# IIT-PAVIS/Acoustic-Image-Generation

Hardware: AMD Instinct MI355X
Metric: train-step images/sec (higher is better)
Workload: dtype f32

## Files before the change

### acoustic-image-generation_amd/acimg/_lib.py

```python
import ctypes as C
import os

_HERE = os.path.dirname(os.path.abspath(__file__))
LIB_PATH = os.environ.get("ACIMG_LIB") or os.path.join(_HERE, "lib", "libacimg.so")

ACT_NONE, ACT_RELU, ACT_SIGMOID = 0, 1, 2


class ConvDesc(C.Structure):

    _fields_ = [(n, C.c_int32) for n in (
        "N", "H", "W", "C", "ldx", "K", "ldy", "OH", "OW", "R", "S", "stride", "pad_t", "pad_l",
        "ldw", "act")]

    def __repr__(self):
        return "ConvDesc(" + ", ".join("%s=%d" % (n, getattr(self, n)) for n, _ in self._fields_) + ")"


class Config(C.Structure):

    _fields_ = [(n, C.c_int32) for n in (
        "splitk_cut", "splitk_target", "splitk_handoff", "wgrad_minpix", "wgrad_halo", "split3_tile_bm",
        "split3_tile_bn", "tail_split", "tail_s", "trunk_persistent", "trunk_bk", "trunk_stagger", "trunk_dma_pos",
        "trunk_ring", "trunk_ring_bm", "trunk_halo")]
# ... 26 lines not shown
    "acimg_last_error": (_I, [C.c_char_p, _SZ]),
    "acimg_conv2d_fwd": (_I, [_DP, _P, _P, _P, _P, _P, _P, _I, _P, _P, _SZ, _P, _P]),
    "acimg_conv2d_stats_rows": (_I, [_DP]),
    "acimg_conv2d_fwd_tiling": (_I, [_DP, C.POINTER(C.c_int)]),
    "acimg_config_default": (_I, [C.POINTER(Config)]),
    "acimg_configure": (_I, [C.POINTER(Config)]),
    "acimg_conv2d_fwd_workspace": (_SZ, [_DP]),
    "acimg_conv2d_split3_weight_bytes": (_SZ, [_DP]),
    "acimg_conv2d_split3_prepare": (_I, [_DP, _P, _P, _P]),
    "acimg_conv2d_bf16_prepare": (_I, [_DP, _P, _P, _P]),
    "acimg_conv2d_fwd_split3_stats_rows": (_I, [_DP]),
    "acimg_conv2d_fwd_split3_tiling": (_I, [_DP, C.POINTER(C.c_int)]),
    "acimg_conv2d_fwd_split3p_stats_rows": (_I, [_DP]),
    "acimg_conv2d_fwd_split3": (_I, [_DP, _P, _P, _P, _P, _P, _P, _I, _P, _P]),
    "acimg_conv2d_fwd_bf16": (_I, [_DP, _P, _P, _P, _P, _P, _P, _I, _P, _P]),
    "acimg_conv2d_split3_dgrad_weight_bytes": (_SZ, [_DP]),
    "acimg_conv2d_split3_prepare_dgrad": (_I, [_DP, _P, _P, _P]),
    "acimg_conv2d_dgrad_split3": (_I, [_DP, _P, _I, _P, _P, _I, _P, _I, _P, _I, _P]),
    "acimg_conv2d_dgrad_bf16": (_I, [_DP, _P, _I, _P, _P, _I, _P, _I, _P, _I, _P]),
    "acimg_conv2d_split3_prepare_multi": (_I, [_I, _P, _P, _P, _P, _P]),
    "acimg_conv2d_fwd_split3p_workspace": (_SZ, [_DP]),
    "acimg_conv2d_fwd_split3p": (_I, [_DP, _P, _SZ, _P, _P, _P, _P, _SZ, _P]),
    "acimg_conv2d_fwd_split1p": (_I, [_DP, _P, _SZ, _P, _P, _P, _P, _SZ, _P]),
    "acimg_conv2d_fwd_split3p_stats": (_I, [_DP, _P, _SZ, _P, _P, _P, _SZ, _P]),
    "acimg_gram_stats_workspace": (_SZ, [_L, _I]),
    "acimg_gram_stats": (_I, [_P, _SZ, _L, _I, _P, _I, _I, _P, _P, _P, _P, _F, _F, _P, _P, _P, _SZ, _P]),
    "acimg_conv2d_fwd_split3p_tail": (_I, [_DP, _P, _SZ, _P, _P, _P, _P, _SZ, _P, _SZ, _P, _SZ, _P]),
    "acimg_conv2d_fwd_split3p_tail_proj": (_I, [_DP, _P, _SZ, _P, _P, _P, _P, _P, _P, _P, _SZ, _P, _SZ, _P]),
    "acimg_split_plane_bytes": (_SZ, [_L, _I]),
    "acimg_bn_relu_split": (_I, [_P, _P, _P, _I, _P, _SZ, _L, _I, _P]),
    "acimg_bn_add_relu_split": (_I, [_P, _P, _P, _P, _P, _P, _P, _SZ, _P, _SZ, _P, _I, _I, _I, _I, _I, _I, _I, _P]),
    "acimg_bn_relu_maxpool_split": (_I, [_P, _P, _P, _P, _SZ, _I, _I, _I, _I, _I, _I, _I, _I, _P]),
    "acimg_conv2d_dgrad": (_I, [_DP, _P, _I, _P, _P, _I, _P, _I, _P, _I, _P, _SZ, _P, _P]),
    "acimg_conv2d_dgrad_workspace": (_SZ, [_DP]),
    "acimg_conv2d_wgrad": (_I, [_DP, _P, _P, _I, _P, _P, _P, _SZ, _P]),
    "acimg_conv2d_wgrad_workspace": (_SZ, [_DP]),
    "acimg_conv2d_wgrad_split3": (_I, [_DP, _P, _P, _I, _P, _P, _P, _SZ, _P]),
    "acimg_conv2d_wgrad_bf16": (_I, [_DP, _P, _P, _I, _P, _P, _P, _SZ, _P]),
    "acimg_conv2d_affine_input_ok": (_I, [_DP, _I]),
    "acimg_conv2d_wgrad_affine": (_I, [_DP, _I, _P, _P, _P, _I, _P, _I, _P, _P, _P, _SZ, _P]),
    "acimg_deconv_fwd": (_I, [_DP, _P, _P, _P, _P, _P, _SZ, _P, _P]),
    "acimg_deconv_dgrad": (_I, [_DP, _P, _I, _P, _P, _P, _I, _P, _SZ, _P, _P]),
    "acimg_deconv_wgrad": (_I, [_DP, _P, _P, _I, _P, _P, _P, _SZ, _P]),
    "acimg_deconv_workspace": (_SZ, [_DP]),
    "acimg_bn_finalize": (_I, [_P, _I, _I, _I, _D, _P, _P, _P, _P, _F, _F, _I, _P, _P, _P, _P, _P]),
    "acimg_bn_add_relu": (_I, [_P, _P, _P, _P, _P, _P, _P, _I, _I, _I, _I, _I, _I, _I, _P]),
# ... 134 lines not shown
```

### acoustic-image-generation_amd/acimg/ops.py

```python
import ctypes as C
import math

import torch

from . import _lib
from ._lib import ACT_NONE, ACT_RELU, ACT_SIGMOID, ConvDesc


def up4(v):
    return (int(v) + 3) & ~3


class Ptr(object):

    __slots__ = ("t", "off")

    def __init__(self, t, off=0):
        self.t = t
        self.off = int(off)

    def addr(self):
        return self.t.data_ptr() + 4 * self.off


# ... 404 lines not shown

def conv2d_fwd_split3(plan, d, x, wsplit, y, in_scale=None, in_shift=None, in_relu=0, stats=None, bias=None, bf16=False):
    fn = _L().acimg_conv2d_fwd_bf16 if bf16 else _L().acimg_conv2d_fwd_split3
    _check_stats_rows(stats, _L().acimg_conv2d_fwd_split3_stats_rows(C.byref(d)), "conv2d_fwd_split3")
    plan.add("conv2d_fwd_bf16" if bf16 else "conv2d_fwd_split3", fn, C.byref(d), x, wsplit, bias, y, in_scale, in_shift,
             int(in_relu), stats)


def conv2d_split3_dgrad_weight_bytes(d):
    return _L().acimg_conv2d_split3_dgrad_weight_bytes(C.byref(d))


def conv2d_split3_prepare_dgrad(plan, d, w, wsplit):
    plan.add("conv2d_split3_prepare_dgrad", _L().acimg_conv2d_split3_prepare_dgrad, C.byref(d), w, wsplit)


def conv2d_dgrad_split3(plan, d, gy, ldgy, wsplit_t, dx, residual=None, ldres=0, mask=None, ldmask=0, lddx=0,
                        bf16=False):
    fn = _L().acimg_conv2d_dgrad_bf16 if bf16 else _L().acimg_conv2d_dgrad_split3
    plan.add("conv2d_dgrad_bf16" if bf16 else "conv2d_dgrad_split3", fn, C.byref(d), gy, int(ldgy), wsplit_t, dx,
             int(lddx), residual, int(ldres), mask, int(ldmask))


def conv2d_fwd_split3p_workspace(d):
    return int(_L().acimg_conv2d_fwd_split3p_workspace(C.byref(d)))


def conv2d_fwd_split3p(plan, d, x_planes, x_lo_off, wsplit, y, stats=None, tail_ws=None, terms=3, side=False):
    nbytes = 0 if tail_ws is None else (tail_ws.numel() * tail_ws.element_size() if hasattr(tail_ws, "numel") else 0)
    fn = _L().acimg_conv2d_fwd_split3p if terms == 3 else _L().acimg_conv2d_fwd_split1p
    plan.add("conv2d_fwd_split3p" if terms == 3 else "conv2d_fwd_split1p", fn, C.byref(d), x_planes, int(x_lo_off),
             wsplit, y, stats, tail_ws, int(nbytes), side=side)


def conv2d_fwd_split3p_stats(plan, d, x_planes, x_lo_off, wsplit, stats, tail_ws=None, side=False):
    nbytes = 0 if tail_ws is None else (tail_ws.numel() * tail_ws.element_size() if hasattr(tail_ws, "numel") else 0)
    plan.add("conv2d_fwd_split3p_stats", _L().acimg_conv2d_fwd_split3p_stats, C.byref(d), x_planes, int(x_lo_off), wsplit,
             stats, tail_ws, int(nbytes), side=side)


def gram_stats_workspace(rows, Cn):
    return int(_L().acimg_gram_stats_workspace(int(rows), int(Cn)))


def gram_stats(plan, x_planes, x_lo_off, rows, Cn, w, ldw, K, gamma, beta, moving_mean, moving_var, scale, shift, ws,
               decay=0.997, eps=1e-5, side=False):
    plan.add("gram_stats", _L().acimg_gram_stats, x_planes, int(x_lo_off), int(rows), int(Cn), w, int(ldw), int(K), gamma,
             beta, moving_mean, moving_var, float(decay), float(eps), scale, shift, ws,
             int(ws.numel() * ws.element_size()), side=side)


def conv2d_fwd_split3p_tail(plan, d, x_planes, x_lo_off, wsplit, scale, shift, sc_planes, sc_lo_off, out_planes,
                            out_lo_off, tail_ws=None, side=False):
    nbytes = 0 if tail_ws is None else (tail_ws.numel() * tail_ws.element_size() if hasattr(tail_ws, "numel") else 0)
    plan.add("conv2d_fwd_split3p_tail", _L().acimg_conv2d_fwd_split3p_tail, C.byref(d), x_planes, int(x_lo_off), wsplit,
             scale, shift, sc_planes, int(sc_lo_off), out_planes, int(out_lo_off), tail_ws, int(nbytes), side=side)

# ... 324 lines not shown
```

### acoustic-image-generation_amd/acimg/unet_acresnet.py

```python
import os
from collections import OrderedDict

import numpy as np
import torch

from . import ops
from .ops import ACT_NONE, ACT_RELU, ACT_SIGMOID, Ptr
from .params import FusedHeads, Var, up4
from .session import get_default_session
from .vision import load_state_file

Z = 150


class Act(object):

    def __init__(self, t, N, H, W, C, ld=None, off=0):
        self.t, self.N, self.H, self.W, self.C = t, N, H, W, C
        self.ld = up4(C) if ld is None else ld
        self.off = off

    @property
    def ptr(self):
        return Ptr(self.t, self.off)

    @property
    def Cp(self):
        return up4(self.C)

    @property
    def pixels(self):
        return self.N * self.H * self.W


class UNetAc(object):

    def __init__(self, input_shape=None, num_frames=12, embedding=False, num_skip=1, precision="split", side_lane=True):
        assert precision in ("split", "f32")
        self.precision = precision
        self.split_min_rows = 16384
        self.side_lane = bool(side_lane)
        self._wsplit_bufs = {}
        self.scope = 'UNetAcRes'
        self.num_frames = num_frames
        self.height = input_shape[0]
        self.width = input_shape[1]
        self.channels = input_shape[2]
        self.embedding = bool(embedding)
        self.num_skip = int(num_skip)
        assert self.num_skip in (0, 1, 2)
        self.session = None

    def _conv_specs(self):
        ns = self.num_skip
        return OrderedDict([
            ("final", (3, 3, 64, 12)),
            ("layer7/conv_2", (3, 3, 64, 64)), ("layer7/conv_1", (3, 3, 128, 64)),
            ("layer6/conv_2", (3, 3, 128, 128)), ("layer6/conv_1", (3, 3, 128 if ns == 0 else 256, 128)),
            ("layer5/conv_2", (3, 3, 128, 128)), ("layer5/conv_1", (3, 3, 128, 128)),
            ("layer4/conv_2", (3, 3, 128, 128)), ("layer4/conv_1", (3, 3, 266 if ns == 2 else 133, 128)),
            ("conv2d", (3, 3, 12, 133)),
            ("layer2/conv_2", (3, 3, 133, 133)), ("layer2/conv_1", (3, 3, 128, 133)),
            ("layer1/pool_2", (3, 3, 128, 128)), ("layer1/conv_2", (3, 3, 128, 128)),
# ... 110 lines not shown
        else:
            self.mean = self.zbuf[:, :Z]
        self.output = self.yhat.t
        self.network = OrderedDict(input=acoustic_images, is_training=None, keep_prob=None,
                                   features=self.cat145[..., :145])
        self.train_vars = [n for n in sess.store.tf_names() if n.startswith(self.scope + "/")]

    def _P(self, name):
        st = self.session.store
        return ops.LazyPtr(lambda: st.p(self.scope + "/" + name))

    def _G(self, name):
        st = self.session.store
        return ops.LazyPtr(lambda: st.g(self.scope + "/" + name))

    def _desc(self, x, K, stride=1, y=None, act=ACT_NONE):
        return ops.conv_desc(x.N, x.H, x.W, x.Cp if x.off == 0 and x.ld == x.Cp else x.C, K, 3, 3, stride, "SAME",
                             ldx=x.ld, ldy=(y.ld if y is not None else up4(K)), ldw=up4(K), act=act)

    def _use_split(self, d):
        return (self.precision == "split" and d.stride == 1 and d.C % 32 == 0 and d.K % 32 == 0 and
                d.N * d.OH * d.OW >= self.split_min_rows)

    def _wsplit(self, name, nbytes, kind):
        key = (name, kind)
        if key not in self._wsplit_bufs:
            self._wsplit_bufs[key] = torch.zeros(int(nbytes), dtype=torch.uint8, device=self.session.device)
        return self._wsplit_bufs[key]

    def _prepare_job(self, plan, d, name, image, mode):
        if getattr(self, "_prep_jobs", None) is None:
            (ops.conv2d_split3_prepare_dgrad if mode else ops.conv2d_split3_prepare)(plan, d, self._P(name + "/kernel"),
                                                                                      image)
            return
        self._prep_jobs.add(d, self._P(name + "/kernel"), image, mode)

    def _conv(self, plan, name, x, y, stride=1, act=ACT_RELU):
        d = self._desc(x, y.C, stride, y, act)
        self._descs[name] = (d, x, y)
        if self._use_split(d):
            ws = self._wsplit(name, ops.conv2d_split3_weight_bytes(d), "fwd")
            self._prepare_job(plan, d, name, ws, 0)
            ops.conv2d_fwd_split3(plan, d, x.ptr, ws, y.ptr, bias=self._P(name + "/bias"))
        else:
            ops.conv2d_fwd(plan, d, x.ptr, self._P(name + "/kernel"), self._P(name + "/bias"), y.ptr)

    def _record_forward(self, plan):
        N = self.N
        self._descs = {}
        h, w = self.pool1.H, self.pool1.W
        self._prep_jobs = None
        if self.precision == "split":
            self._prep_jobs = ops.PrepareJobs()
            ops.conv2d_split3_prepare_multi(plan, self._prep_jobs)
        self._conv(plan, "layer1/conv_1", self.inp, self.c11)
        self._conv(plan, "layer1/conv_2", self.c11, self.conv1)
        self._conv(plan, "layer1/pool_2", self.conv1, self.pool1, stride=3)
        self._conv(plan, "layer2/conv_1", self.pool1, self.c21)
        self._conv(plan, "layer2/conv_2", self.c21, self.conv2_0)
        ops.minmax_fwd(plan, self.conv2_0.ptr, self.conv2_0.ld, self.cat145, 148, self.mm_a, N, h * w, 133)
        ops.minmax_fwd(plan, self.feat.ptr, 12, Ptr(self.cat145, 133), 148, self.mm_b, N, h * w, 12)
        kin = h * w * 148
        self.d_heads = ops.conv_desc(N, 1, 1, kin, self.hn if not self.embedding else Z, 1, 1, 1, "VALID",
                                     ldx=kin, ldy=self.hn, ldw=self.hn)
        ops.conv2d_fwd(plan, self.d_heads, self.cat145, self._P("heads/kernel"), self._P("heads/bias"),
                       self.heads_out)
        if self.embedding:
            ops.minmax_fwd(plan, self.heads_out, self.hn, self.zbuf, 152, self.mm_z, N, 1, Z)
        else:
            ops.latent_fwd(plan, self.heads_out, self.eps, self.zbuf, 152, self.sigma, self.kl, N, Z)
        self.d_dense = ops.conv_desc(N, 1, 1, 152, 2304, 1, 1, 1, "VALID", ldx=152, ldy=2304, ldw=2304,
                                     act=ACT_RELU)
        ops.conv2d_fwd(plan, self.d_dense, self.zbuf, self._P("dense/kernel"), self._P("dense/bias"), self.dns.t)
        self._conv(plan, "conv2d", self.dns, self.net)
        self._conv(plan, "layer4/conv_1", self.l4in, self.c41)
        self._conv(plan, "layer4/conv_2", self.c41, self.conv4)
        self._conv(plan, "layer5/conv_1", self.conv4, self.c51)
        self._conv(plan, "layer5/conv_2", self.c51, self.conv5)
        self.d_up = ops.deconv_desc(N, h, w, 128, 128, 2, 2, 3, ldx=128, ldy=self.up.ld, ldw=128)
        ops.deconv_fwd(plan, self.d_up, self.conv5.ptr, self._P("upsample_1/kernel"), self._P("upsample_1/bias"),
                       self.up.ptr)
        self._conv(plan, "layer6/conv_1", self.l6in, self.c61)
        self._conv(plan, "layer6/conv_2", self.c61, self.conv6)
        self._conv(plan, "layer7/conv_1", self.conv6, self.c71)
        self._conv(plan, "layer7/conv_2", self.c71, self.conv7)
        self._conv(plan, "final", self.conv7, self.yhat, act=ACT_SIGMOID)

    def record_backward(self, plan, g_logit, g_feat, kl_weight, on_ready=None):
        on_ready = on_ready or (lambda name: None)
        N = self.N
        z = self.session.zeros
        H, W, h, w = self.height, self.width, self.pool1.H, self.pool1.W
        ns = self.num_skip

        def gbuf(a, full=False):
            return Act(z(a.N, a.H, a.W, up4(a.C)), a.N, a.H, a.W, a.C)

        def back(name, gy, dx=None, mask=None, res=None):
            d, x, y = self._descs[name]
            wg = ops.conv2d_wgrad_split3 if (self.precision == "split" and d.K % 64 == 0) else ops.conv2d_wgrad
            beside = dx is not None and self.side_lane
            if beside:
                plan.fork()
            wg(plan, d, x.ptr, gy.ptr, gy.ld, self._G(name + "/kernel"), self._G(name + "/bias"), side=beside)
            if dx is not None and self._use_split(d):
                wt = self._wsplit(name, ops.conv2d_split3_dgrad_weight_bytes(d), "dgrad")
                self._prepare_job(plan, d, name, wt, 1)
# ... 78 lines not shown
```

### acoustic-image-generation_amd/csrc/igemm.hip

```cpp
#include "wgrad_split3_kernel.hpp"
#include "igemm_split3d_kernel.hpp"
#include "igemm_split3dp_kernel.hpp"
#include "igemm_split3r_kernel.hpp"
#include "igemm_split3h_kernel.hpp"
#include "skinny_kernel.hpp"
#include <cstdlib>
#include <algorithm>
#include <type_traits>

namespace acimg {

__global__ __launch_bounds__(256) void igemm_splitk_reduce_kernel(const float* slab, int splits,
                                                                  int M, int Ngemm, int slab_ld,
                                                                  const EpiParams e) {
    const long idx = (long)blockIdx.x * 256 + threadIdx.x;
    const long total = (long)M * Ngemm;
    if (idx >= total) return;
    const int m = (int)(idx / Ngemm);
    const int n = (int)(idx - (long)m * Ngemm);
    float v = 0.f;
    for (int z = 0; z < splits; ++z) v += slab[((long)z * M + m) * slab_ld + n];
    if (n >= e.Nstore) return;
    int cn, pixoff, r, q, oh, ow;
    epi_col(e, n, cn, pixoff, r, q);
// ... 2633 lines not shown
    if (rc) return rc;
    if (d->K % 32 || d->K > d->ldw) return fail(ACIMG_EINVAL, "conv2d_split3_prepare_dgrad: K must be a multiple of 32");
    const int Ktot = d->R * d->S * d->K;
    hipLaunchKernelGGL((split3_prepare_kernel<SplitBF16, true>), dim3(cdiv(Ktot, 32), cdiv(d->C, 32)), dim3(256), 0,
                       (hipStream_t)stream, w, d->R * d->S, d->C, d->K, d->ldw, d->C, static_cast<__bf16*>(wsplit));
    return check_launch("split3_prepare_dgrad");
}

int acimg_conv2d_split3_prepare_multi(int n, const AcimgConvDesc* const* descs, const float* const* w, void* const* out,
                                      const int* mode, void* stream) {
    if (n == 0) return ACIMG_OK;
    if (n < 0 || n > 16 || !descs || !w || !out || !mode)
        return fail(ACIMG_EINVAL, "conv2d_split3_prepare_multi: need 0..16 jobs and non-null tables");
    PrepJobs jobs{};
    jobs.n = n;
    int blocks = 0;
    for (int i = 0; i < n; ++i) {
        const AcimgConvDesc* d = descs[i];
        int rc = check_desc(d, "conv2d_split3_prepare_multi", true);
        if (rc) return rc;
        if (!w[i] || !out[i]) return fail(ACIMG_EINVAL, "conv2d_split3_prepare_multi: null pointer in job %d", i);
        PrepJob& J = jobs.j[i];
        J.w = w[i]; J.out = out[i]; J.ntaps = d->R * d->S; J.C = d->C; J.K = d->K; J.ldw = d->ldw;
        if (mode[i] < 0 || mode[i] > 2) return fail(ACIMG_EINVAL, "conv2d_split3_prepare_multi: job %d: mode is 0, 1 or 2", i);
        J.dgrad = mode[i];
        int tiles_n;
        if (J.dgrad == 1) {
            if (d->K % 32 || d->K > d->ldw)
                return fail(ACIMG_EINVAL, "conv2d_split3_prepare_multi: job %d: K must be a multiple of 32", i);
            J.Nrows = d->C;
            J.tiles_k = cdiv(d->R * d->S * d->K, 32);
            tiles_n = cdiv(d->C, 32);
        } else {
            J.Nrows = d->ldw;
            J.tiles_k = cdiv(d->R * d->S * d->C, 32);
            tiles_n = cdiv(d->ldw, 32);
        }
        J.block0 = blocks;
        blocks += J.tiles_k * tiles_n;
    }
    hipLaunchKernelGGL(split3_prepare_multi_kernel, dim3(blocks), dim3(256), 0, (hipStream_t)stream, jobs);
    return check_launch("split3_prepare_multi");
}

extern "C++" {
template <typename TR, int TERMS = 3>
static int launch_split3(IgemmParams& p, hipStream_t st) {
    Split3Cfg c = pick_split3(p.M, p.Ngemm, true);
    dim3 grid(cdiv(p.M, c.bm), cdiv(p.Ngemm, c.bn), 1);
    if (c.bm == 128 && c.bn == 32)
        hipLaunchKernelGGL((igemm_split3_kernel<128, 32, 4, 1, 256, TR, TERMS>), grid, dim3(256), 2 * (2 * 128 * 64 + 2 * 32 * 64), st, p);
    else if (c.bm == 128 && c.bn == 128)
        hipLaunchKernelGGL((igemm_split3_kernel<128, 128, 2, 4, 512, TR, TERMS>), grid, dim3(512), 65536, st, p);
    else if (c.bm == 64 && c.bn == 128)
        hipLaunchKernelGGL((igemm_split3_kernel<64, 128, 1, 4, 256, TR, TERMS>), grid, dim3(256), 2 * (2 * 64 * 64 + 2 * 128 * 64), st, p);
    else if (c.bm == 128 && c.bn == 64)
        hipLaunchKernelGGL((igemm_split3_kernel<128, 64, 2, 2, 256, TR, TERMS>), grid, dim3(256), 2 * (2 * 128 * 64 + 2 * 64 * 64), st, p);
    else
        return fail(ACIMG_EINVAL, "split3: unsupported tile %dx%d", c.bm, c.bn);
    return check_launch("igemm_split3");
}

static void epi_vec_flag(EpiParams& e) {
    e.vec = aligned16(e.Y) && (e.ldy & 3) == 0 && (!e.bias || aligned16(e.bias)) &&
            (!e.res || (aligned16(e.res) && (e.ldres & 3) == 0)) &&
// ... 170 lines not shown
extern "C" int acimg_debug_no_output_stores(int on) {
    g_stamp_nostore = on;
    return 0;
}
#endif

size_t acimg_conv2d_fwd_split3p_workspace(const AcimgConvDesc* d) {
    (void)d;
    return TS_COUNTER_BYTES + (size_t)TS_MAX_UNITS * 128 * 128 * sizeof(float);
}

struct Split3pTail {
    int mode;
    const float* scale;
    const float* shift;
    const void* sc_planes;
    size_t sc_lo_off;
    void* out_planes;
    size_t out_lo_off;
    const float* scale2;
    const float* shift2;
};

static int fwd_presplit(const AcimgConvDesc* d, const void* x_planes, size_t x_lo_off, const void* wsplit, float* y,
                        float* stats, void* ws, size_t ws_bytes, void* stream, const int terms,
                        const Split3pTail* tail = nullptr) {
    int rc = check_desc(d, "conv2d_fwd_split3p");
    if (rc) return rc;
    if (d->C % 32) return fail(ACIMG_EINVAL, "conv2d_fwd_split3p: C=%d must be a multiple of 32", d->C);
    if (d->ldw < d->K || !aligned16(x_planes) || !aligned16(wsplit) || !aligned16(y) || (d->ldy & 3) || d->ldx != d->C ||
        (x_lo_off & 15))
        return fail(ACIMG_EINVAL, "conv2d_fwd_split3p: ldw<K, ldx != C (split-format tensors are dense) or unaligned operands");
    IgemmParams p{};
    p.A = static_cast<const float*>(x_planes); p.H = d->H; p.W = d->W; p.C = d->C; p.lda = d->ldx;
    p.OH = d->OH; p.OW = d->OW; p.R = d->R; p.S = d->S; p.stride = d->stride;
    p.pad_t = d->pad_t; p.pad_l = d->pad_l;
    p.M = d->N * d->OH * d->OW;
    p.B = static_cast<const float*>(wsplit); p.Nld = d->ldw; p.Ngemm = d->K;
    p.ntaps = d->R * d->S;
    p.kiters = p.ntaps * (d->C / 32);
    p.splits = 1;
    const long plane = (long)acimg_split_plane_bytes((long)d->N * d->H * d->W, d->C);
    const long a_bytes = (long)x_lo_off + plane;
    const long b_bytes = (long)acimg_conv2d_split3_weight_bytes(d);
    if (a_bytes >= (1L << 31) || b_bytes >= (1L << 31) || (long)x_lo_off < plane)
        return fail(ACIMG_EINVAL, "conv2d_fwd_split3p: operand >= 2 GiB or overlapping planes");
    p.a_bytes = (unsigned)a_bytes; p.b_bytes = (unsigned)b_bytes; p.a_lo_off = (unsigned)x_lo_off;
    p.b_brick = (unsigned)split3_rowmajor_bytes(d);
    EpiParams& e = p.e;
// ... 34 lines not shown
        }
        const long oplane = (long)acimg_split_plane_bytes((long)p.M, d->K);
        if (!aligned16(tail->sc_planes) || !aligned16(tail->out_planes) || (tail->out_lo_off & 15) ||
            (long)tail->out_lo_off < oplane || (long)tail->out_lo_off + oplane >= (1L << 31))
            return fail(ACIMG_EINVAL, "conv2d_fwd_split3p_tail: unaligned / overlapping / >= 2 GiB split-format operands");
        e.Y = nullptr; e.stats = nullptr;
        e.f_scale = tail->scale; e.f_shift = tail->shift;
        e.f_sc = static_cast<const char*>(tail->sc_planes);
        e.f_out = static_cast<char*>(tail->out_planes); e.f_out_lo = (unsigned)tail->out_lo_off;
        e.f_out_bytes = (unsigned)(tail->out_lo_off + oplane);
        if (tail->mode == 3) {
            e.f_scale2 = tail->scale2; e.f_shift2 = tail->shift2;
            e.f_sc_lo = 0; e.f_sc_bytes = (unsigned)((long)p.M * d->K * 4);
            hipLaunchKernelGGL((igemm_split3dp_kernel<32, 0, 3, 3>), dim3(nwg), dim3(512), lds_t, st, p, units, nwg);
            return check_launch("conv2d_fwd_split3p_tail_proj");
        }
        if ((tail->sc_lo_off & 15) || (long)tail->sc_lo_off < oplane || (long)tail->sc_lo_off + oplane >= (1L << 31))
            return fail(ACIMG_EINVAL, "conv2d_fwd_split3p_tail: unaligned / overlapping / >= 2 GiB shortcut planes");
        e.f_sc_lo = (unsigned)tail->sc_lo_off;
        e.f_sc_bytes = (unsigned)(tail->sc_lo_off + oplane);
        hipLaunchKernelGGL((igemm_split3dp_kernel<32, 0, 3, 2>), dim3(nwg), dim3(512), lds_t, st, p, units, nwg);
        return check_launch("conv2d_fwd_split3p_tail");
    }
    if (halo_on(d, terms)) {
        const size_t lds_h = (size_t)2 * (HALO_NB * 1024 + 64) + 2 * 2 * 128 * 64;
        const void* fh = (const void*)igemm_split3h_kernel<HALO_NB>;
        static bool attr_h = false;
        if (!attr_h) {
            (void)hipFuncSetAttribute(fh, hipFuncAttributeMaxDynamicSharedMemorySize, (int)lds_h);
            attr_h = true;
        }
        const int Ph = resident_slots(7, fh, 512, lds_h);
        TailPlan th{T, 1, 0};
        if (ws && ws_bytes >= acimg_conv2d_fwd_split3p_workspace(d)) th = pick_tail(T, Ph, p.kiters, TS_MAX_UNITS);
        p.ts_whole = th.whole; p.ts_s = th.s;
        p.ts_counters = static_cast<int*>(ws);
        p.ts_partial = ws ? reinterpret_cast<float*>(static_cast<char*>(ws) + TS_COUNTER_BYTES) : nullptr;
        hipLaunchKernelGGL((igemm_split3h_kernel<HALO_NB>), dim3(th.whole + th.rem * th.s), dim3(512), lds_h, st, p);
        return check_launch("conv2d_fwd_split3p (halo)");
    }
    if (const int rr = big_out ? 0 : ring_rows(d, terms)) {
#if defined(ACIMG_STAMP) || defined(ACIMG_ABLATE)
        p.slab = g_stamp_buf;
        p.flip = g_stamp_nostore;
#endif
        p.ras_tiles_m = cdiv(p.M, rr);
// ... 47 lines not shown
            hipLaunchKernelGGL((igemm_split3dp_kernel<32, 0>), dim3(nwg), dim3(512), lds_p, st, p, n_units, nwg);
        }
    } else if (terms == 1) {
        if (which == 0)
            hipLaunchKernelGGL((igemm_split3d_kernel<128, 128, 2, 4, 512, 2, 2, 1>), grid, dim3(512), lds_bytes, st, p);
        else if (which == 1)
            hipLaunchKernelGGL((igemm_split3d_kernel<64, 128, 1, 4, 256, 2, 2, 1>), grid, dim3(256), lds_bytes, st, p);
        else
            hipLaunchKernelGGL((igemm_split3d_kernel<128, 64, 2, 2, 256, 2, 2, 1>), grid, dim3(256), lds_bytes, st, p);
    } else if (which == 0)
        hipLaunchKernelGGL((igemm_split3d_kernel<128, 128, 2, 4, 512, 2, 2>), grid, dim3(512), lds_bytes, st, p);
    else if (which == 1)
        hipLaunchKernelGGL((igemm_split3d_kernel<64, 128, 1, 4, 256, 2, 2>), grid, dim3(256), lds_bytes, st, p);
    else
        hipLaunchKernelGGL((igemm_split3d_kernel<128, 64, 2, 2, 256, 2, 2>), grid, dim3(256), lds_bytes, st, p);
    return check_launch("conv2d_fwd_split3p");
}

int acimg_conv2d_fwd_split3p(const AcimgConvDesc* d, const void* x_planes, size_t x_lo_off, const void* wsplit,
                             float* y, float* stats, void* ws, size_t ws_bytes, void* stream) {
    return fwd_presplit(d, x_planes, x_lo_off, wsplit, y, stats, ws, ws_bytes, stream, 3);
}

int acimg_conv2d_fwd_split1p(const AcimgConvDesc* d, const void* x_planes, size_t x_lo_off, const void* wsplit,
                             float* y, float* stats, void* ws, size_t ws_bytes, void* stream) {
    return fwd_presplit(d, x_planes, x_lo_off, wsplit, y, stats, ws, ws_bytes, stream, 1);
}

int acimg_conv2d_fwd_split3p_stats(const AcimgConvDesc* d, const void* x_planes, size_t x_lo_off, const void* wsplit,
                                   float* stats, void* ws, size_t ws_bytes, void* stream) {
    if (!stats) return fail(ACIMG_EINVAL, "conv2d_fwd_split3p_stats: null statistics buffer");
    const Split3pTail t{1, nullptr, nullptr, nullptr, 0, nullptr, 0, nullptr, nullptr};
    return fwd_presplit(d, x_planes, x_lo_off, wsplit, nullptr, stats, ws, ws_bytes, stream, 3, &t);
}

int acimg_conv2d_fwd_split3p_tail(const AcimgConvDesc* d, const void* x_planes, size_t x_lo_off, const void* wsplit,
                                  const float* scale, const float* shift, const void* sc_planes, size_t sc_lo_off,
                                  void* out_planes, size_t out_lo_off, void* ws, size_t ws_bytes, void* stream) {
    if (!scale || !shift || !sc_planes || !out_planes || !aligned16(scale) || !aligned16(shift))
        return fail(ACIMG_EINVAL, "conv2d_fwd_split3p_tail: null / unaligned scale, shift, shortcut or output");
    const Split3pTail t{2, scale, shift, sc_planes, sc_lo_off, out_planes, out_lo_off, nullptr, nullptr};
    return fwd_presplit(d, x_planes, x_lo_off, wsplit, nullptr, nullptr, ws, ws_bytes, stream, 3, &t);
}

int acimg_conv2d_fwd_split3p_tail_proj(const AcimgConvDesc* d, const void* x_planes, size_t x_lo_off, const void* wsplit,
                                       const float* scale, const float* shift, const float* sc32, const float* sc_scale,
// ... 122 lines not shown
```

### acoustic-image-generation_amd/csrc/igemm_split3d_kernel.hpp

```cpp
#pragma once
#include "igemm_split3_kernel.hpp"

namespace acimg {

typedef __attribute__((address_space(3))) void* lds_ptr_t;

__device__ __forceinline__ unsigned brick_a_off(unsigned f, unsigned c32, unsigned kc) {
    return (f >> 4) * c32 + ((f & 15u) << 6) + (((kc ^ (0u - (f >> 2))) & 3u) << 4);
}
__device__ __forceinline__ unsigned brick_b_off(unsigned n, unsigned ksteps, unsigned pch) {
    return (n >> 7) * ksteps * 16384u + ((n & 127u) << 6) + (pch << 4);
}

template <int N>
__device__ __forceinline__ void wait_vmcnt() {
    static_assert(N >= 0 && N < 64, "vmcnt immediate");
    if constexpr (N == 0) asm volatile("s_waitcnt vmcnt(0)" ::: "memory");
    else if constexpr (N == 1) asm volatile("s_waitcnt vmcnt(1)" ::: "memory");
    else if constexpr (N == 2) asm volatile("s_waitcnt vmcnt(2)" ::: "memory");
    else if constexpr (N == 3) asm volatile("s_waitcnt vmcnt(3)" ::: "memory");
    else if constexpr (N == 4) asm volatile("s_waitcnt vmcnt(4)" ::: "memory");
    else if constexpr (N == 6) asm volatile("s_waitcnt vmcnt(6)" ::: "memory");
    else if constexpr (N == 8) asm volatile("s_waitcnt vmcnt(8)" ::: "memory");
    else if constexpr (N == 9) asm volatile("s_waitcnt vmcnt(9)" ::: "memory");
    else if constexpr (N == 10) asm volatile("s_waitcnt vmcnt(10)" ::: "memory");
    else if constexpr (N == 12) asm volatile("s_waitcnt vmcnt(12)" ::: "memory");
    else static_assert(N == 0, "add the immediate");
}

__device__ __forceinline__ void raster_tile(const IgemmParams& p, int L, int& mt, int& nt) {
    const int T = p.ras_tiles_m * p.ras_tiles_n;
    const int xcd = L & 7, slot = L >> 3;
    const int base = T >> 3, extra = T & 7;
    const int ord = xcd * base + min(xcd, extra) + slot;
    const int band = p.ras_gm * p.ras_tiles_n;
    const int mband = ord / band;
    const int rem = ord - mband * band;
    const int gm = min(p.ras_gm, p.ras_tiles_m - mband * p.ras_gm);
    const int grp = gm * p.ras_gn;
    const int ngroup = rem / grp;
    const int r2 = rem - ngroup * grp;
    const int gn = min(p.ras_gn, p.ras_tiles_n - ngroup * p.ras_gn);
    const int mi = r2 / gn;
    mt = mband * p.ras_gm + mi;
    nt = ngroup * p.ras_gn + (r2 - mi * gn);
}

template <int BM, int BN, int WGM, int WGN, int NTHR, int NSA, int NSB, int TERMS = 3>
__global__ __launch_bounds__(NTHR) void igemm_split3d_kernel(const IgemmParams p) {
    constexpr int BK = 32;
    constexpr int ROWB = BK * 2;
    constexpr int A_BYTES = BM * ROWB;
    constexpr int B_BYTES = BN * ROWB;
    constexpr int B_BASE = NSA * 2 * A_BYTES;
    constexpr int WTM = BM / WGM, WTN = BN / WGN;
    constexpr int TM = WTM / 16, TN = WTN / 16;
    constexpr int NW = NTHR / 64;
    constexpr int RA = BM / 16 / NW;
    constexpr int RB = BN / 16 / NW;
    constexpr int INFLIGHT = (NSB - 2) * 2 * (RA + RB) + (NSA - NSB) * 2 * RA;
    static_assert(WGM * WGN == NW && (BM / 16) % NW == 0 && (BN / 16) % NW == 0, "tile / wave mapping");
    static_assert(NSB >= 2 && (NSA == NSB || NSA == NSB + 1), "stage counts");

    extern __shared__ __attribute__((aligned(16))) float smem[];
    char* const lds = reinterpret_cast<char*>(smem);

    const int tid = threadIdx.x;
    const int lane = tid & 63, wid = tid >> 6;
    const int wm = wid / WGN, wn = wid % WGN;
    const int li = lane & 15, g = lane >> 4;
    int vt = blockIdx.x, chunk = 0;
// ... 194 lines not shown
                __hip_atomic_store(p.ts_counters + tl, 0, __ATOMIC_RELAXED, __HIP_MEMORY_SCOPE_AGENT);
            }
            *flag = last;
        }
        __syncthreads();
        if (!*flag) return;
        __syncthreads();
#pragma unroll
        for (int i = 0; i < TM; ++i)
#pragma unroll
            for (int j = 0; j < TN; ++j) acc[i][j] = f32x4{0.f, 0.f, 0.f, 0.f};
        for (int c = 0; c < p.ts_s; ++c) {
            const __amdgpu_buffer_rsrc_t rsQ =
                __builtin_amdgcn_make_buffer_rsrc(slot0 + (long)c * (BM * BN), 0, BM * BN * 4, 0x00020000);
#pragma unroll
            for (int i = 0; i < TM; ++i)
#pragma unroll
                for (int j = 0; j < TN; ++j)
                    acc[i][j] += __builtin_bit_cast(f32x4, __builtin_amdgcn_raw_buffer_load_b128(
                                                               rsQ, ((i * TN + j) * NTHR + tid) * 16, 0, 16));
        }
    }
    const EpiParams& e = p.e;
    if (e.vec && !e.bias && !e.res && !e.mask && !e.scatter && e.act == ACIMG_ACT_NONE) {
        constexpr int CH = BN / 4;
        f32x4* tile = reinterpret_cast<f32x4*>(smem);
        float* red = smem + BM * BN;
        if (e.stats) {
#pragma unroll
            for (int j = 0; j < TN; ++j) {
                f32x4 s1 = acc[0][j], s2 = acc[0][j] * acc[0][j];
#pragma unroll
                for (int i = 1; i < TM; ++i) {
                    s1 += acc[i][j];
                    s2 += acc[i][j] * acc[i][j];
                }
#pragma unroll
                for (int k = 0; k < 4; ++k) {
                    s1[k] = row16_sum(s1[k]);
                    s2[k] = row16_sum(s2[k]);
                }
                if (li == 0) {
                    const int n = wn * WTN + j * 16 + g * 4;
                    *reinterpret_cast<f32x4*>(red + (wm * 2 + 0) * BN + n) = s1;
                    *reinterpret_cast<f32x4*>(red + (wm * 2 + 1) * BN + n) = s2;
                }
            }
        }
#pragma unroll
        for (int i = 0; i < TM; ++i) {
            const int row = wm * WTM + i * 16 + li;
// ... 8 lines not shown
        static_assert(BM * CH % NTHR == 0, "row store mapping");
#pragma unroll
        for (int t0 = 0; t0 < NIT; t0 += 4) {
            f32x4 v[4];
#pragma unroll
            for (int k = 0; k < 4; ++k) {
                const int t = tid + (t0 + k) * NTHR;
                const int row = t / CH, c = t - row * CH;
                v[k] = tile[row * CH + (c ^ (row & (CH - 1)))];
            }
#pragma unroll
            for (int k = 0; k < 4; ++k) {
                const int t = tid + (t0 + k) * NTHR;
                const int row = t / CH, c = t - row * CH;
                const int m = m0 + row, n = n0 + 4 * c;
                if (m < e.M && n < e.Nstore) {
                    float* dst = e.Y + (long)m * e.ldy + n;
                    if (n + 3 < e.Nstore) *reinterpret_cast<f32x4*>(dst) = v[k];
                    else
                        for (int q = 0; q < 4 && n + q < e.Nstore; ++q) dst[q] = v[k][q];
                }
            }
        }
        if (e.stats) {
            for (int idx = tid; idx < 2 * BN; idx += NTHR) {
                const int which = idx / BN, c = idx - which * BN;
                const int n = n0 + c;
                if (n < e.stats_ld) {
                    float sum = 0.f;
#pragma unroll
                    for (int w = 0; w < WGM; ++w) sum += red[(w * 2 + which) * BN + c];
                    e.stats[((long)mt * 2 + which) * e.stats_ld + n] = sum;
                }
            }
        }
        return;
    }
    igemm_epilogue<BM, BN, WGM, WGN, NTHR, TM, TN>(p, acc, smem, m0, n0, wm, wn, li, g, tid, mt);
}

}
```

### include/acimg.h

```cpp
#ifndef ACIMG_H_
#define ACIMG_H_

#include <stddef.h>
#include <stdint.h>

#ifdef __cplusplus
extern "C" {
#endif

#define ACIMG_VERSION 207

#define ACIMG_OK 0
#define ACIMG_EINVAL (-1)
#define ACIMG_EWORKSPACE (-2)
#define ACIMG_ELAUNCH (-3)

#define ACIMG_ACT_NONE 0
#define ACIMG_ACT_RELU 1
#define ACIMG_ACT_SIGMOID 2

int acimg_version(void);
int acimg_last_error(char* buf, size_t len);

typedef struct AcimgConvDesc {
// ... 42 lines not shown
int acimg_conv2d_fwd_split3(const AcimgConvDesc* d, const float* x, const void* wsplit, const float* bias,
                            float* y, const float* in_scale, const float* in_shift, int in_relu, float* stats,
                            void* stream);
size_t acimg_conv2d_split3_dgrad_weight_bytes(const AcimgConvDesc* d);
int acimg_conv2d_split3_prepare_dgrad(const AcimgConvDesc* d, const float* w, void* wsplit, void* stream);
int acimg_conv2d_dgrad_split3(const AcimgConvDesc* d, const float* gy, int ldgy, const void* wsplit_t, float* dx,
                              int lddx, const float* residual, int ldres, const float* mask, int ldmask,
                              void* stream);

int acimg_conv2d_bf16_prepare(const AcimgConvDesc* d, const float* w, void* wsplit, void* stream);
int acimg_conv2d_fwd_bf16(const AcimgConvDesc* d, const float* x, const void* wsplit, const float* bias,
                          float* y, const float* in_scale, const float* in_shift, int in_relu, float* stats,
                          void* stream);
int acimg_conv2d_dgrad_bf16(const AcimgConvDesc* d, const float* gy, int ldgy, const void* wsplit_t, float* dx,
                            int lddx, const float* residual, int ldres, const float* mask, int ldmask,
                            void* stream);

size_t acimg_conv2d_fwd_split3p_workspace(const AcimgConvDesc* d);
int acimg_conv2d_fwd_split3p_stats_rows(const AcimgConvDesc* d);
int acimg_conv2d_fwd_split3p(const AcimgConvDesc* d, const void* x_planes, size_t x_lo_off, const void* wsplit,
                             float* y, float* stats, void* ws, size_t ws_bytes, void* stream);
int acimg_conv2d_fwd_split1p(const AcimgConvDesc* d, const void* x_planes, size_t x_lo_off, const void* wsplit,
                             float* y, float* stats, void* ws, size_t ws_bytes, void* stream);
int acimg_conv2d_fwd_split3p_stats(const AcimgConvDesc* d, const void* x_planes, size_t x_lo_off, const void* wsplit,
                                   float* stats, void* ws, size_t ws_bytes, void* stream);
int acimg_conv2d_fwd_split3p_tail(const AcimgConvDesc* d, const void* x_planes, size_t x_lo_off, const void* wsplit,
                                  const float* scale, const float* shift, const void* sc_planes, size_t sc_lo_off,
                                  void* out_planes, size_t out_lo_off, void* ws, size_t ws_bytes, void* stream);
int acimg_conv2d_fwd_split3p_tail_proj(const AcimgConvDesc* d, const void* x_planes, size_t x_lo_off, const void* wsplit,
                                       const float* scale, const float* shift, const float* sc32, const float* sc_scale,
                                       const float* sc_shift, void* out_planes, size_t out_lo_off, void* ws, size_t ws_bytes,
                                       void* stream);
size_t acimg_gram_stats_workspace(long rows, int C);
int acimg_gram_stats(const void* x_planes, size_t x_lo_off, long rows, int C, const float* w, int ldw, int K,
                     const float* gamma, const float* beta, float* moving_mean, float* moving_var, float decay, float eps,
                     float* scale, float* shift, void* ws, size_t ws_bytes, void* stream);
size_t acimg_split_plane_bytes(long rows, int C);
int acimg_bn_relu_split(const float* x, const float* scale, const float* shift, int relu, void* out,
                        size_t lo_off, long rows, int C, void* stream);
int acimg_bn_add_relu_split(const float* a, const float* sa, const float* ta, const float* b32,
                            const float* sb, const float* tb, const void* b_planes, size_t b_lo_off,
                            void* out_planes, size_t out_lo_off, float* out32, int N, int OH, int OW, int C,
                            int BH, int BW, int bstride, void* stream);
int acimg_bn_relu_maxpool_split(const float* x, const float* scale, const float* shift, void* out,
                                size_t lo_off, int N, int H, int W, int C, int OH, int OW, int pad_t, int pad_l,
                                void* stream);
// ... 190 lines not shown
```

Before: 5042.

## Chain UNet decoder convs through pre-split fp16 planes with fused bias/ReLU epilogue

Adds a split3p_act forward path that reads the input as pre-split hi/lo fp16 planes and applies bias and ReLU in the epilogue. The epilogue can also write the output directly as split planes for the next conv, so the decoder convs in layers 6 and 7 chain without re-splitting the fp32 activation inside each conv. It uses a tile-order weight image (prepare mode 3) and ping-pong plane buffers. The aim is to cut the per-conv split/convert work and global reads. The cost is an extra standalone split pass at the start of each chain and extra plane memory.

```diff
diff --git a/acoustic-image-generation_amd/acimg/_lib.py b/acoustic-image-generation_amd/acimg/_lib.py
--- a/acoustic-image-generation_amd/acimg/_lib.py
+++ b/acoustic-image-generation_amd/acimg/_lib.py
@@ -72,6 +72,7 @@
     "acimg_conv2d_fwd_split3p_workspace": (_SZ, [_DP]),
     "acimg_conv2d_fwd_split3p": (_I, [_DP, _P, _SZ, _P, _P, _P, _P, _SZ, _P]),
     "acimg_conv2d_fwd_split1p": (_I, [_DP, _P, _SZ, _P, _P, _P, _P, _SZ, _P]),
+    "acimg_conv2d_fwd_split3p_act": (_I, [_DP, _P, _SZ, _P, _P, _P, _P, _SZ, _P, _SZ, _P]),
     "acimg_conv2d_fwd_split3p_stats": (_I, [_DP, _P, _SZ, _P, _P, _P, _SZ, _P]),
     "acimg_gram_stats_workspace": (_SZ, [_L, _I]),
     "acimg_gram_stats": (_I, [_P, _SZ, _L, _I, _P, _I, _I, _P, _P, _P, _P, _F, _F, _P, _P, _P, _SZ, _P]),
diff --git a/acoustic-image-generation_amd/acimg/ops.py b/acoustic-image-generation_amd/acimg/ops.py
--- a/acoustic-image-generation_amd/acimg/ops.py
+++ b/acoustic-image-generation_amd/acimg/ops.py
@@ -450,6 +450,10 @@
              int(lddx), residual, int(ldres), mask, int(ldmask))
 
 
+def split_plane_bytes(rows, Cn):
+    return int(_L().acimg_split_plane_bytes(int(rows), int(Cn)))
+
+
 def conv2d_fwd_split3p_workspace(d):
     return int(_L().acimg_conv2d_fwd_split3p_workspace(C.byref(d)))
 
@@ -461,6 +465,13 @@
              wsplit, y, stats, tail_ws, int(nbytes), side=side)
 
 
+def conv2d_fwd_split3p_act(plan, d, x_planes, x_lo_off, wsplit, y, bias=None, out_planes=None, out_lo_off=0, tail_ws=None,
+                          side=False):
+    nbytes = 0 if tail_ws is None else (tail_ws.numel() * tail_ws.element_size() if hasattr(tail_ws, "numel") else 0)
+    plan.add("conv2d_fwd_split3p_act", _L().acimg_conv2d_fwd_split3p_act, C.byref(d), x_planes, int(x_lo_off), wsplit,
+             bias, y, out_planes, int(out_lo_off), tail_ws, int(nbytes), side=side)
+
+
 def conv2d_fwd_split3p_stats(plan, d, x_planes, x_lo_off, wsplit, stats, tail_ws=None, side=False):
     nbytes = 0 if tail_ws is None else (tail_ws.numel() * tail_ws.element_size() if hasattr(tail_ws, "numel") else 0)
     plan.add("conv2d_fwd_split3p_stats", _L().acimg_conv2d_fwd_split3p_stats, C.byref(d), x_planes, int(x_lo_off), wsplit,
diff --git a/acoustic-image-generation_amd/acimg/unet_acresnet.py b/acoustic-image-generation_amd/acimg/unet_acresnet.py
--- a/acoustic-image-generation_amd/acimg/unet_acresnet.py
+++ b/acoustic-image-generation_amd/acimg/unet_acresnet.py
@@ -35,10 +35,14 @@
 
 class UNetAc(object):
 
-    def __init__(self, input_shape=None, num_frames=12, embedding=False, num_skip=1, precision="split", side_lane=True):
+    def __init__(self, input_shape=None, num_frames=12, embedding=False, num_skip=1, precision="split", side_lane=True,
+                 planes_min_rows=55296):
         assert precision in ("split", "f32")
         self.precision = precision
         self.split_min_rows = 16384
+        self.planes_min_rows = planes_min_rows
+        self._plane_bufs = {}
+        self._plane_of = {}
         self.side_lane = bool(side_lane)
         self._wsplit_bufs = {}
         self.scope = 'UNetAcRes'
@@ -195,6 +199,27 @@
         return (self.precision == "split" and d.stride == 1 and d.C % 32 == 0 and d.K % 32 == 0 and
                 d.N * d.OH * d.OW >= self.split_min_rows)
 
+    def _use_planes(self, d, x):
+        return (self._use_split(d) and self.num_skip == 1 and self.planes_min_rows is not None and d.R == 3 and
+                d.S == 3 and d.C % 32 == 0 and d.K % 64 == 0 and x.off == 0 and x.ld == x.C and
+                d.N * d.OH * d.OW >= self.planes_min_rows)
+
+    def _planes(self, slot, a):
+        lo = ops.split_plane_bytes(a.pixels, a.C)
+        cap = 2 * ops.split_plane_bytes(a.pixels, 128 if slot else 256)
+        assert 2 * lo <= cap
+        key = (slot, a.pixels)
+        if key not in self._plane_bufs:
+            self._plane_bufs[key] = torch.zeros(cap, dtype=torch.uint8, device=self.session.device)
+        return self._plane_bufs[key], lo
+
+    def _identity_affine(self, C):
+        key = ("planes/affine", C)
+        if key not in self._wsplit_bufs:
+            dev = self.session.device
+            self._wsplit_bufs[key] = (torch.ones(C, device=dev), torch.zeros(C, device=dev))
+        return self._wsplit_bufs[key]
+
     def _wsplit(self, name, nbytes, kind):
         key = (name, kind)
         if key not in self._wsplit_bufs:
@@ -208,10 +233,27 @@
             return
         self._prep_jobs.add(d, self._P(name + "/kernel"), image, mode)
 
-    def _conv(self, plan, name, x, y, stride=1, act=ACT_RELU):
+    def _conv(self, plan, name, x, y, stride=1, act=ACT_RELU, planes_out=False):
         d = self._desc(x, y.C, stride, y, act)
         self._descs[name] = (d, x, y)
-        if self._use_split(d):
+        if self._use_planes(d, x):
+            ws = self._wsplit(name, ops.conv2d_split3_weight_bytes(d), "fwd")
+            self._prepare_job(plan, d, name, ws, 3)
+            if self._plane_of.get("tensor") is not x:
+                slot = 0
+                xp, xlo = self._planes(slot, x)
+                one, zero = self._identity_affine(x.C)
+                ops.bn_relu_split(plan, x.ptr, one, zero, 0, xp, xlo, x.pixels, x.C)
+            else:
+                slot = self._plane_of["slot"]
+                xp, xlo = self._planes(slot, x)
+            yp, ylo = (None, 0)
+            if planes_out:
+                yp, ylo = self._planes(slot ^ 1, y)
+                self._plane_of = {"tensor": y, "slot": slot ^ 1}
+            ops.conv2d_fwd_split3p_act(plan, d, xp, xlo, ws, y.ptr, bias=self._P(name + "/bias"), out_planes=yp,
+                                       out_lo_off=ylo)
+        elif self._use_split(d):
             ws = self._wsplit(name, ops.conv2d_split3_weight_bytes(d), "fwd")
             self._prepare_job(plan, d, name, ws, 0)
             ops.conv2d_fwd_split3(plan, d, x.ptr, ws, y.ptr, bias=self._P(name + "/bias"))
@@ -223,6 +265,7 @@
         self._descs = {}
         h, w = self.pool1.H, self.pool1.W
         self._prep_jobs = None
+        self._plane_of = {}
         if self.precision == "split":
             self._prep_jobs = ops.PrepareJobs()
             ops.conv2d_split3_prepare_multi(plan, self._prep_jobs)
@@ -253,9 +296,9 @@
         self.d_up = ops.deconv_desc(N, h, w, 128, 128, 2, 2, 3, ldx=128, ldy=self.up.ld, ldw=128)
         ops.deconv_fwd(plan, self.d_up, self.conv5.ptr, self._P("upsample_1/kernel"), self._P("upsample_1/bias"),
                        self.up.ptr)
-        self._conv(plan, "layer6/conv_1", self.l6in, self.c61)
-        self._conv(plan, "layer6/conv_2", self.c61, self.conv6)
-        self._conv(plan, "layer7/conv_1", self.conv6, self.c71)
+        self._conv(plan, "layer6/conv_1", self.l6in, self.c61, planes_out=True)
+        self._conv(plan, "layer6/conv_2", self.c61, self.conv6, planes_out=True)
+        self._conv(plan, "layer7/conv_1", self.conv6, self.c71, planes_out=True)
         self._conv(plan, "layer7/conv_2", self.c71, self.conv7)
         self._conv(plan, "final", self.conv7, self.yhat, act=ACT_SIGMOID)
 
diff --git a/acoustic-image-generation_amd/csrc/igemm.hip b/acoustic-image-generation_amd/csrc/igemm.hip
--- a/acoustic-image-generation_amd/csrc/igemm.hip
+++ b/acoustic-image-generation_amd/csrc/igemm.hip
@@ -2679,8 +2679,10 @@
         if (!w[i] || !out[i]) return fail(ACIMG_EINVAL, "conv2d_split3_prepare_multi: null pointer in job %d", i);
         PrepJob& J = jobs.j[i];
         J.w = w[i]; J.out = out[i]; J.ntaps = d->R * d->S; J.C = d->C; J.K = d->K; J.ldw = d->ldw;
-        if (mode[i] < 0 || mode[i] > 2) return fail(ACIMG_EINVAL, "conv2d_split3_prepare_multi: job %d: mode is 0, 1 or 2", i);
-        J.dgrad = mode[i];
+        if (mode[i] < 0 || mode[i] > 3) return fail(ACIMG_EINVAL, "conv2d_split3_prepare_multi: job %d: mode is 0 .. 3", i);
+        if (mode[i] == 3 && !split3_brick_bytes(d))
+            return fail(ACIMG_EINVAL, "conv2d_split3_prepare_multi: job %d: the tile-order image needs C %% 32 == 0", i);
+        J.dgrad = mode[i] == 3 ? 0 : mode[i];
         int tiles_n;
         if (J.dgrad == 1) {
             if (d->K % 32 || d->K > d->ldw)
@@ -2697,7 +2699,17 @@
         blocks += J.tiles_k * tiles_n;
     }
     hipLaunchKernelGGL(split3_prepare_multi_kernel, dim3(blocks), dim3(256), 0, (hipStream_t)stream, jobs);
-    return check_launch("split3_prepare_multi");
+    int rc = check_launch("split3_prepare_multi");
+    for (int i = 0; i < n && !rc; ++i) {
+        if (mode[i] != 3) continue;
+        const AcimgConvDesc* d = descs[i];
+        const long total = (long)(split3_brick_bytes(d) / 16);
+        hipLaunchKernelGGL(split3_brick_kernel, dim3((unsigned)cdiv(total, 256L)), dim3(256), 0, (hipStream_t)stream,
+                           static_cast<const char*>(out[i]), static_cast<char*>(out[i]) + split3_rowmajor_bytes(d), d->ldw,
+                           d->R * d->S * d->C, total);
+        rc = check_launch("split3_prepare_multi (tile order)");
+    }
+    return rc;
 }
 
 extern "C++" {
@@ -2914,9 +2926,15 @@
     const float* shift2;
 };
 
+struct Split3pAct {
+    const float* bias;
+    void* out_planes;
+    size_t out_lo_off;
+};
+
 static int fwd_presplit(const AcimgConvDesc* d, const void* x_planes, size_t x_lo_off, const void* wsplit, float* y,
                         float* stats, void* ws, size_t ws_bytes, void* stream, const int terms,
-                        const Split3pTail* tail = nullptr) {
+                        const Split3pTail* tail = nullptr, const Split3pAct* actp = nullptr) {
     int rc = check_desc(d, "conv2d_fwd_split3p");
     if (rc) return rc;
     if (d->C % 32) return fail(ACIMG_EINVAL, "conv2d_fwd_split3p: C=%d must be a multiple of 32", d->C);
@@ -2997,6 +3015,38 @@
         hipLaunchKernelGGL((igemm_split3dp_kernel<32, 0, 3, 2>), dim3(nwg), dim3(512), lds_t, st, p, units, nwg);
         return check_launch("conv2d_fwd_split3p_tail");
     }
+    if (actp) {
+        if (d->stride != 1 || d->K % 64 || (d->act != ACIMG_ACT_NONE && d->act != ACIMG_ACT_RELU) || !y || d->ldy < d->K ||
+            !aligned16(actp->bias))
+            return fail(ACIMG_EINVAL, "conv2d_fwd_split3p_act: needs stride 1, K %% 64 == 0, act none / ReLU, aligned bias");
+        e.bias = actp->bias;
+        e.stats = nullptr;
+        if (actp->out_planes) {
+            const size_t oplane = acimg_split_plane_bytes((long)p.M, d->K);
+            if (!aligned16(actp->out_planes) || (actp->out_lo_off & 15) || actp->out_lo_off < oplane ||
+                actp->out_lo_off + oplane >= ((size_t)1 << 32))
+                return fail(ACIMG_EINVAL, "conv2d_fwd_split3p_act: unaligned / overlapping / >= 4 GiB output planes");
+            e.f_out = static_cast<char*>(actp->out_planes);
+            e.f_out_lo = (unsigned)actp->out_lo_off;
+        }
+        const void* fa = which == 0 ? (const void*)igemm_split3d_kernel<128, 128, 2, 4, 512, 2, 2, 3, true>
+                       : which == 1 ? (const void*)igemm_split3d_kernel<64, 128, 1, 4, 256, 2, 2, 3, true>
+                                    : (const void*)igemm_split3d_kernel<128, 64, 2, 2, 256, 2, 2, 3, true>;
+        TailPlan ta{T, 1, 0};
+        if (ws && ws_bytes >= acimg_conv2d_fwd_split3p_workspace(d) && which == 0)
+            ta = pick_tail(T, resident_slots(11, fa, 512, lds_bytes), p.kiters, TS_MAX_UNITS);
+        p.ts_whole = ta.whole; p.ts_s = ta.s;
+        p.ts_counters = static_cast<int*>(ws);
+        p.ts_partial = ws ? reinterpret_cast<float*>(static_cast<char*>(ws) + TS_COUNTER_BYTES) : nullptr;
+        const dim3 ga(ta.whole + ta.rem * ta.s);
+        if (which == 0)
+            hipLaunchKernelGGL((igemm_split3d_kernel<128, 128, 2, 4, 512, 2, 2, 3, true>), ga, dim3(512), lds_bytes, st, p);
+        else if (which == 1)
+            hipLaunchKernelGGL((igemm_split3d_kernel<64, 128, 1, 4, 256, 2, 2, 3, true>), ga, dim3(256), lds_bytes, st, p);
+        else
+            hipLaunchKernelGGL((igemm_split3d_kernel<128, 64, 2, 2, 256, 2, 2, 3, true>), ga, dim3(256), lds_bytes, st, p);
+        return check_launch("conv2d_fwd_split3p_act");
+    }
     if (halo_on(d, terms)) {
         const size_t lds_h = (size_t)2 * (HALO_NB * 1024 + 64) + 2 * 2 * 128 * 64;
         const void* fh = (const void*)igemm_split3h_kernel<HALO_NB>;
@@ -3090,6 +3140,13 @@
     return fwd_presplit(d, x_planes, x_lo_off, wsplit, y, stats, ws, ws_bytes, stream, 3);
 }
 
+int acimg_conv2d_fwd_split3p_act(const AcimgConvDesc* d, const void* x_planes, size_t x_lo_off, const void* wsplit,
+                                 const float* bias, float* y, void* out_planes, size_t out_lo_off, void* ws, size_t ws_bytes,
+                                 void* stream) {
+    const Split3pAct a{bias, out_planes, out_lo_off};
+    return fwd_presplit(d, x_planes, x_lo_off, wsplit, y, nullptr, ws, ws_bytes, stream, 3, nullptr, &a);
+}
+
 int acimg_conv2d_fwd_split1p(const AcimgConvDesc* d, const void* x_planes, size_t x_lo_off, const void* wsplit,
                              float* y, float* stats, void* ws, size_t ws_bytes, void* stream) {
     return fwd_presplit(d, x_planes, x_lo_off, wsplit, y, stats, ws, ws_bytes, stream, 1);
diff --git a/acoustic-image-generation_amd/csrc/igemm_split3d_kernel.hpp b/acoustic-image-generation_amd/csrc/igemm_split3d_kernel.hpp
--- a/acoustic-image-generation_amd/csrc/igemm_split3d_kernel.hpp
+++ b/acoustic-image-generation_amd/csrc/igemm_split3d_kernel.hpp
@@ -46,7 +46,7 @@
     nt = ngroup * p.ras_gn + (r2 - mi * gn);
 }
 
-template <int BM, int BN, int WGM, int WGN, int NTHR, int NSA, int NSB, int TERMS = 3>
+template <int BM, int BN, int WGM, int WGN, int NTHR, int NSA, int NSB, int TERMS = 3, bool ACT = false>
 __global__ __launch_bounds__(NTHR) void igemm_split3d_kernel(const IgemmParams p) {
     constexpr int BK = 32;
     constexpr int ROWB = BK * 2;
@@ -287,11 +287,27 @@
         }
     }
     const EpiParams& e = p.e;
-    if (e.vec && !e.bias && !e.res && !e.mask && !e.scatter && e.act == ACIMG_ACT_NONE) {
+    if (ACT || (e.vec && !e.bias && !e.res && !e.mask && !e.scatter && e.act == ACIMG_ACT_NONE)) {
         constexpr int CH = BN / 4;
         f32x4* tile = reinterpret_cast<f32x4*>(smem);
         float* red = smem + BM * BN;
-        if (e.stats) {
+        if constexpr (ACT) {
+#pragma unroll
+            for (int j = 0; j < TN; ++j) {
+                const int n = n0 + wn * WTN + j * 16 + g * 4;
+                f32x4 b = f32x4{0.f, 0.f, 0.f, 0.f};
+                if (e.bias && n < e.Nstore) b = *reinterpret_cast<const f32x4*>(e.bias + n);
+#pragma unroll
+                for (int i = 0; i < TM; ++i) {
+                    acc[i][j] += b;
+                    if (e.act == ACIMG_ACT_RELU) {
+#pragma unroll
+                        for (int k = 0; k < 4; ++k) acc[i][j][k] = fmaxf(acc[i][j][k], 0.f);
+                    }
+                }
+            }
+        }
+        if (!ACT && e.stats) {
 #pragma unroll
             for (int j = 0; j < TN; ++j) {
                 f32x4 s1 = acc[0][j], s2 = acc[0][j] * acc[0][j];
@@ -346,6 +362,35 @@
                 }
             }
         }
+        if constexpr (ACT) {
+            if (e.f_out) {
+                const unsigned CQ = (unsigned)e.Nstore >> 5;
+                const unsigned kc = (((unsigned)lane & 3u) ^ (0u - ((unsigned)lane >> 4))) & 3u;
+                for (int b = wid; b < (BM / 16) * (BN / 32); b += NW) {
+                    const int pg = b / (BN / 32), cgl = b - pg * (BN / 32);
+                    const int lr = pg * 16 + (lane >> 2);
+                    const int cl = cgl * 32 + (int)kc * 8;
+                    const int c4 = cl >> 2;
+                    const f32x4 v0 = tile[lr * CH + (c4 ^ (lr & (CH - 1)))];
+                    const f32x4 v1 = tile[lr * CH + ((c4 + 1) ^ (lr & (CH - 1)))];
+                    if (m0 + lr < e.M && n0 + cl < e.Nstore) {
+                        h16x8 oh, ol;
+#pragma unroll
+                        for (int k = 0; k < 8; ++k) {
+                            const float o = (k < 4 ? v0[k & 3] : v1[k & 3]) * SPLIT3_ASCALE;
+                            const _Float16 hh = (_Float16)o;
+                            oh[k] = hh;
+                            ol[k] = (_Float16)(o - (float)hh);
+                        }
+                        char* dst = e.f_out + ((size_t)((unsigned)(m0 + pg * 16) >> 4) * CQ + (unsigned)((n0 >> 5) + cgl)) * 1024u +
+                                    (unsigned)lane * 16u;
+                        *reinterpret_cast<h16x8*>(dst) = oh;
+                        *reinterpret_cast<h16x8*>(dst + e.f_out_lo) = ol;
+                    }
+                }
+            }
+            return;
+        }
         if (e.stats) {
             for (int idx = tid; idx < 2 * BN; idx += NTHR) {
                 const int which = idx / BN, c = idx - which * BN;
diff --git a/include/acimg.h b/include/acimg.h
--- a/include/acimg.h
+++ b/include/acimg.h
@@ -88,6 +88,9 @@
                              float* y, float* stats, void* ws, size_t ws_bytes, void* stream);
 int acimg_conv2d_fwd_split1p(const AcimgConvDesc* d, const void* x_planes, size_t x_lo_off, const void* wsplit,
                              float* y, float* stats, void* ws, size_t ws_bytes, void* stream);
+int acimg_conv2d_fwd_split3p_act(const AcimgConvDesc* d, const void* x_planes, size_t x_lo_off, const void* wsplit,
+                                 const float* bias, float* y, void* out_planes, size_t out_lo_off, void* ws, size_t ws_bytes,
+                                 void* stream);
 int acimg_conv2d_fwd_split3p_stats(const AcimgConvDesc* d, const void* x_planes, size_t x_lo_off, const void* wsplit,
                                    float* stats, void* ws, size_t ws_bytes, void* stream);
 int acimg_conv2d_fwd_split3p_tail(const AcimgConvDesc* d, const void* x_planes, size_t x_lo_off, const void* wsplit,
```

New measurement: 5096 (median of 2 runs). No clear change (+1.1%).
